# mcan1999/vulkan-raytracing

Measured on AMD Instinct MI355X. Metric: Mrays/sec (primary+secondary) at 1920×1080 depth 4; 1/2/4/8-GPU scaling, higher is better.
Workload: dtype f32

## Files before the change

### vulkan_raytracing_amd/csrc/kernels.hip

```cpp
#include <hip/hip_runtime.h>

#include "rt_kernels.h"

namespace rt {

struct F3 { float x, y, z; };
__device__ __forceinline__ F3 mk3(float x, float y, float z) { F3 r; r.x = x; r.y = y; r.z = z; return r; }
__device__ __forceinline__ F3 add3(F3 a, F3 b) { return mk3(a.x + b.x, a.y + b.y, a.z + b.z); }
__device__ __forceinline__ F3 sub3(F3 a, F3 b) { return mk3(a.x - b.x, a.y - b.y, a.z - b.z); }
__device__ __forceinline__ F3 mul3(F3 a, float s) { return mk3(a.x * s, a.y * s, a.z * s); }
__device__ __forceinline__ F3 neg3(F3 a) { return mk3(-a.x, -a.y, -a.z); }
__device__ __forceinline__ float dot3(F3 a, F3 b) { return __builtin_fmaf(a.z, b.z, __builtin_fmaf(a.y, b.y, a.x * b.x)); }
__device__ __forceinline__ F3 cross3(F3 a, F3 b) {
  return mk3(__builtin_fmaf(a.y, b.z, -(a.z * b.y)), __builtin_fmaf(a.z, b.x, -(a.x * b.z)), __builtin_fmaf(a.x, b.y, -(a.y * b.x)));
}
__device__ __forceinline__ float length3(F3 v) { return __builtin_sqrtf(dot3(v, v)); }
__device__ __forceinline__ F3 normalize3(F3 v) { float inv = 1.0f / length3(v); return mul3(v, inv); }
__device__ __forceinline__ F3 fma3(float s, F3 a, F3 b) { return mk3(__builtin_fmaf(s, a.x, b.x), __builtin_fmaf(s, a.y, b.y), __builtin_fmaf(s, a.z, b.z)); }
__device__ __forceinline__ F3 reflect3(F3 I, F3 N) { float k = 2.0f * dot3(N, I); return fma3(-k, N, I); }

__device__ __forceinline__ F3 xform_point(const float* m, F3 p) {
  return mk3(__builtin_fmaf(m[2], p.z, __builtin_fmaf(m[1], p.y, m[0] * p.x)) + m[3],
             __builtin_fmaf(m[6], p.z, __builtin_fmaf(m[5], p.y, m[4] * p.x)) + m[7],
             __builtin_fmaf(m[10], p.z, __builtin_fmaf(m[9], p.y, m[8] * p.x)) + m[11]);
// ... 1260 lines not shown
      atomicAdd(reinterpret_cast<unsigned long long*>(a.counters + CNT_NODE_VISITS + off), (unsigned long long)cnt_nodes);
      atomicAdd(reinterpret_cast<unsigned long long*>(a.counters + CNT_TRI_TESTS + off), (unsigned long long)cnt_tris);
      const int dg = ANY ? CNT_DIAG_SH : CNT_DIAG;
      atomicAdd(reinterpret_cast<unsigned long long*>(a.counters + dg), (unsigned long long)diag_iters);
      atomicAdd(reinterpret_cast<unsigned long long*>(a.counters + dg + 2), (unsigned long long)diag_busy);
      atomicAdd(reinterpret_cast<unsigned long long*>(a.counters + dg + 4), (unsigned long long)(__builtin_readcyclecounter() - diag_t0));
    }
  }
}

template <int MODE, bool ANY, bool WIDE, bool ENTRY = false, bool FAR = true, bool CONT = false>
__global__ __launch_bounds__(256) __attribute__((amdgpu_waves_per_eu(RT_WAVES_PER_EU, RT_WAVES_PER_EU))) void k_trace(TraceArgs a) { trace_body<MODE, ANY, false, WIDE, ENTRY, FAR, CONT>(a); }
template <int MODE, bool ANY, bool WIDE, bool ENTRY = false, bool FAR = true, bool CONT = false>
__global__ __launch_bounds__(256) void k_trace_count(TraceArgs a) { trace_body<MODE, ANY, true, WIDE, ENTRY, FAR, CONT>(a); }

#include "kernels_beam.inc"

#ifdef RT_ALT_KERNELS
#include "kernels_alt.inc"
#include "kernels_tile.inc"
#endif

struct ShadeArgs {
  SceneDev sc;
  FrameDev f;
  UniformsDev u;
  int bounce;
  BatchTab bt;
};

struct Surface { F3 P, N; };
__device__ __forceinline__ Surface hit_surface(const SceneDev& sc, const InstanceDev* I, uint32_t prim, float hu, float hv) {
  const uint32_t* ix = sc.idx + I->first_index + 3u * prim;
  const uint32_t ia = ix[0], ib = ix[1], ic = ix[2];
  const float* vb = sc.verts + I->first_float;
  const float bx = (1.0f - hu) - hv, by = hu, bz = hv;
  const float* pa = vb + 6u * ia; const float* pb = vb + 6u * ib; const float* pc = vb + 6u * ic;
  const F3 pos = fma3(bz, mk3(pc[0], pc[1], pc[2]), fma3(by, mk3(pb[0], pb[1], pb[2]), mul3(mk3(pa[0], pa[1], pa[2]), bx)));
  const F3 nrm = fma3(bz, mk3(pc[3], pc[4], pc[5]), fma3(by, mk3(pb[3], pb[4], pb[5]), mul3(mk3(pa[3], pa[4], pa[5]), bx)));
  Surface s;
  s.P = xform_point(I->o2w, pos);
  s.N = normalize3(xform_normal(I->w2o, nrm));
  return s;
}

template <bool TILE = false, bool BATCH = false, bool RUNS = false>
__device__ __forceinline__ void shade_body(const ShadeArgs& a, const int bounce) {
  const FrameDev& f = a.f;
  const UniformsDev& U = a.u;
  const int cur = bounce & 1, nxt = cur ^ 1;
  const uint32_t lane = threadIdx.x & 63u, wave = threadIdx.x >> 6;
  const int n_pass = TILE ? 2 : 1;
  for (int pass = 0; pass < n_pass; pass++) {
  uint32_t cnt[N_SHARDS], maxb = 0;
#pragma unroll
  for (int t = 0; t < N_SHARDS; t++) {
    if (TILE && pass) {
      uint32_t blobs = 0;
#pragma unroll
      for (int k = 0; k < BLOB_CLASSES; k++) blobs += ld_cursor(f.counters + cnt_tail(Q_BLOB_LIST + k, t));
      cnt[t] = blobs * (256u * ((U.samples_per_pixel + 3u) / 4u));
    } else cnt[t] = ld_cursor(f.counters + cnt_tail(bounce, t));
    maxb = max(maxb, (cnt[t] + 63u) >> 6);
  }
  const uint32_t n_waves = gridDim.x * 4u;
  for (uint32_t g = blockIdx.x * 4u + wave; g < maxb * N_SHARDS; g += n_waves) {
    const uint32_t shard = g & (N_SHARDS - 1), base = (g >> 3) << 6;
    uint32_t n = 0;
#pragma unroll
    for (int t = 0; t < N_SHARDS; t++) n = (shard == (uint32_t)t) ? cnt[t] : n;
    if (base >= n) continue;
    const uint32_t q = shard * f.shard_cap + ((TILE && pass) ? f.shard_cap - n : 0u) + base + lane;
    bool push_next = false, push_shadow = false, settled = false;
    F3 no = mk3(0, 0, 0), nd = mk3(0, 0, 1);
    float sh_tmax = 0.f; F3 sh_c = mk3(0, 0, 0); float sh_w = 0.f;
    uint32_t sh_ent = ENTRY_FROM_ROOT;
    uint32_t sid = SID_DEAD;
    int inst = HIT_DEAD;
    if (base + lane < n) inst = ld_stream(&f.hit_inst[q]);
    if (inst != HIT_DEAD) {
      const float4 rd = ld_stream(&f.ray_d[cur][q]);
      sid = __float_as_uint(rd.w);
      const F3 d = mk3(rd.x, rd.y, rd.z);
      if (inst < 0) {
        const F3 c = sample_sky(a.sc, mk3(d.x, d.y, -d.z));
        st_stream(&f.sample_color[sid], make_float4(c.x, c.y, c.z, 1.0f));
      } else {
        const float4 h = ld_stream(&f.hit_a[q]);
        const InstanceDev* I = a.sc.inst + inst;
        const uint32_t prim = __float_as_uint(h.w);
        const Surface S = hit_surface(a.sc, I, prim, h.y, h.z);
        const F3 P = S.P;
        F3 N = S.N;
        const int objectIndex = I->custom_index;
        uint32_t type = I->type != TYPE_BY_OBJECT_INDEX ? I->type : (objectIndex == 0 ? U.center_object_type : U.orbiting_object_type);
        const MaterialDev* M = nullptr;
        uint32_t mat = MATERIAL_NONE;
        if (a.sc.n_materials != 0) {
          mat = a.sc.prim_material[I->first_index / 3u + prim];
          M = a.sc.materials + mat;
          if (M->type != TYPE_BY_INSTANCE) type = M->type;
        }
        const bool last = (uint32_t)bounce >= U.max_bounce_count;
        if (type == 0u) {
          if (dot3(d, N) >= 0.0f) {
            st_stream(&f.sample_color[sid], make_float4(0.08f, 0.24f, 0.08f, 1.0f));
          } else {
            no = fma3(0.01f, N, P);
            F3 light = mk3(U.light_position[0], U.light_position[1], U.light_position[2]);
            float Iv = U.light_intensity;
            uint32_t fi = 0;
            if (BATCH) { fi = frame_of(sid, a.sc.batch_samples); light = mk3(a.bt.light[fi][0], a.bt.light[fi][1], a.bt.light[fi][2]); Iv = a.bt.light[fi][3]; }
            const F3 toL = sub3(light, P);
            const float dist = length3(toL);
            const F3 L = mul3(toL, 1.0f / dist);
            const F3 Hh = normalize3(add3(L, neg3(d)));
            const float NdotL = dot3(N, L), NdotH = dot3(N, Hh);
            const float dl = fmaxf(0.0f, NdotL);
            const float sp = M ? pow_int(fmaxf(0.0f, NdotH), (uint32_t)M->ns) : pow100(fmaxf(0.0f, NdotH));
            const uint32_t i = sid / (uint32_t)(f.rows * f.width) - fi * U.samples_per_pixel;
            float w = 1.0f;
            for (uint32_t k = 0; k < i; k++) w = w * 0.9f;
            const F3 kd = M ? mk3(M->kd[0], M->kd[1], M->kd[2]) : mk3(0.2f, 1.0f, 0.2f);
            const F3 ks = M ? mk3(M->ks[0], M->ks[1], M->ks[2]) : mk3(0.8f, 0.8f, 0.8f);
            const F3 diff = mk3((Iv * kd.x) * dl, (Iv * kd.y) * dl, (Iv * kd.z) * dl);
            const F3 spec = mk3((Iv * ks.x) * sp, (Iv * ks.y) * sp, (Iv * ks.z) * sp);
            const F3 amb = ambient_of(a.sc, mat);
            sh_c = fma3(w, add3(diff, spec), amb); sh_w = __uint_as_float(mat);
            nd = L; sh_tmax = dist;
            push_shadow = true;
            if (f.settle_dead_shadow_rays && __float_as_uint(sh_c.x) == __float_as_uint(amb.x) && __float_as_uint(sh_c.y) == __float_as_uint(amb.y) &&
                __float_as_uint(sh_c.z) == __float_as_uint(amb.z)) {
              st_stream(&f.sample_color[sid], make_float4(amb.x, amb.y, amb.z, 1.0f));
              push_shadow = false; settled = true;
            }
            if (f.light_entry != nullptr) {
              const F3 v = sub3(no, light);
              const float ax = __builtin_fabsf(v.x), ay = __builtin_fabsf(v.y), az = __builtin_fabsf(v.z);
              const int axis = (ax >= ay && ax >= az) ? 0 : (ay >= az ? 1 : 2);
              const float vc = axis == 0 ? v.x : (axis == 1 ? v.y : v.z), va = axis == 0 ? v.y : (axis == 1 ? v.z : v.x), vb = axis == 0 ? v.z : (axis == 1 ? v.x : v.y);
              const float c = __builtin_fabsf(vc);
              if (c > 0.0f) {
                const float T8 = (float)(8 * f.light_tiles);
                const float px = (va / c + 1.0f) * 0.5f * T8, py = (1.0f - vb / c) * 0.5f * T8;
                const int tx = min(max((int)(px * 0.125f), 0), f.light_tiles - 1), ty = min(max((int)(py * 0.125f), 0), f.light_tiles - 1);
                const int face = 2 * axis + (vc < 0.0f ? 1 : 0);
                sh_ent = (uint32_t)((face * f.light_tiles + ty) * f.light_tiles + tx) | (NdotL < 0.0f ? ENTRY_REVERSE : 0u);
              }
            }
          }
        } else if (type == 1u) {
          no = fma3(0.01f, N, P);
          nd = reflect3(d, N);
          push_next = true;
        } else if (type == 2u) {
          float ndoti = dot3(d, N);
          const bool outwards = ndoti > 0.0f;
          if (outwards) { N = neg3(N); ndoti = -ndoti; }
          const float ratio = M ? (outwards ? M->ni : 1.0f / M->ni) : (outwards ? 1.52f : (1.0f / 1.52f));
          const float k = 1.0f - (ratio * ratio) * (1.0f - ndoti * ndoti);
          if (k < 0.0f) { nd = reflect3(d, N); no = fma3(0.01f, N, P); }
          else {
            const float c = __builtin_fmaf(ratio, ndoti, __builtin_sqrtf(k));
            nd = normalize3(fma3(-c, N, mul3(d, ratio)));
            no = fma3(-0.01f, N, P);
          }
          push_next = true;
        } else {
          if (bounce == 0 && f.pixel_runs) {
            no = mk3(U.position[0], U.position[1], U.position[2]);
            if (BATCH) { const uint32_t fk = frame_of(sid, a.sc.batch_samples); no = mk3(a.bt.position[fk][0], a.bt.position[fk][1], a.bt.position[fk][2]); }
          } else {
            const float4 ro = ld_stream(&f.ray_o[cur][q]);
            no = mk3(ro.x, ro.y, ro.z);
          }
          nd = d; push_next = true;
        }
        if (push_next && last) {
          push_next = false;
          st_stream(&f.sample_color[sid], make_float4(0.08f, 0.24f, 0.08f, 1.0f));
        }
      }
    }
    {
      const uint64_t m_st = __ballot(settled);
      if (lane == 0 && m_st != 0ull) {
        __hip_atomic_fetch_add(f.counters + cnt_tail(Q_SHADOW0, (int)shard), (uint32_t)__builtin_popcountll(m_st), __ATOMIC_RELAXED, __HIP_MEMORY_SCOPE_AGENT);
        __hip_atomic_fetch_add(f.counters + cnt_work(Q_DEAD, (int)shard), (uint32_t)__builtin_popcountll(m_st), __ATOMIC_RELAXED, __HIP_MEMORY_SCOPE_AGENT);
      }
    }
    const uint32_t slot_n = wave_alloc(push_next, f.counters + cnt_tail(bounce + 1, (int)shard));
    if (push_next) {
      const uint32_t v = shard * f.shard_cap + slot_n;
      st_stream(&f.ray_o[nxt][v], make_float4(no.x, no.y, no.z, 10000.0f));
      st_stream(&f.ray_d[nxt][v], make_float4(nd.x, nd.y, nd.z, __uint_as_float(sid)));
    }
    if (RUNS) {
      if (base + lane < n) {
        if (push_shadow) {
          st_stream(&f.sh_o[q], make_float4(no.x, no.y, no.z, sh_tmax));
          st_stream(&f.sh_c[q], make_float4(sh_c.x, sh_c.y, sh_c.z, sh_w));
          if (f.sh_e != nullptr) f.sh_e[q] = sh_ent;
        }
        st_stream(&f.sh_d[q], push_shadow ? make_float4(nd.x, nd.y, nd.z, __uint_as_float(sid)) : make_float4(0.f, 0.f, 0.f, __uint_as_float(SID_DEAD)));
      }
      const uint64_t m_sh = __ballot(push_shadow);
      if (lane == 0 && m_sh != 0ull) __hip_atomic_fetch_add(f.counters + cnt_tail(Q_SHADOW0, (int)shard), (uint32_t)__builtin_popcountll(m_sh), __ATOMIC_RELAXED, __HIP_MEMORY_SCOPE_AGENT);
    } else {
      const uint32_t slot_s = wave_alloc(push_shadow, f.counters + cnt_tail(Q_SHADOW, (int)shard));
      if (push_shadow) {
        const uint32_t v = f.sh_base + shard * f.shard_cap + slot_s;
        st_stream(&f.sh_o[v], make_float4(no.x, no.y, no.z, sh_tmax));
        st_stream(&f.sh_d[v], make_float4(nd.x, nd.y, nd.z, __uint_as_float(sid)));
        st_stream(&f.sh_c[v], make_float4(sh_c.x, sh_c.y, sh_c.z, sh_w));
        if (f.sh_e != nullptr) f.sh_e[v] = sh_ent;
      }
    }
  }
  }
}

template <bool TILE, bool BATCH, bool RUNS = false>
__global__ __launch_bounds__(256) void k_shade(ShadeArgs a) { shade_body<TILE, BATCH, RUNS>(a, a.bounce); }

struct TailArgs {
  TraceArgs tr;
  ShadeArgs sh;
  uint32_t first_bounce;
  uint32_t* barrier;
  uint32_t* fault;
};

__device__ __forceinline__ void grid_barrier(uint32_t* bar, uint32_t* fault, uint32_t& phase) {
  __syncthreads();
  phase++;
  if (threadIdx.x == 0) {
    __threadfence();
    const uint32_t target = phase * gridDim.x;
// ... 200 lines not shown
    a.rays_per_lane = (uint32_t)cfg.rays_per_lane; a.min_blocks = (uint32_t)cfg.min_blocks;
    const dim3 g(cfg.trace_blocks), b(256);
#ifdef RT_ALT_KERNELS
    if (f.tile_blob != nullptr) {
      if (counting) hipLaunchKernelGGL((k_trace_count<MODE_CLOSEST, false, false, true, false, true>), g, b, 0, s, a);
      else hipLaunchKernelGGL((k_trace<MODE_CLOSEST, false, false, true, false, true>), g, b, 0, s, a);
      return;
    }
#endif
    if (counting) hipLaunchKernelGGL((k_trace_count<MODE_CLOSEST, false, false, true>), g, b, 0, s, a);
    else if (cfg.far) hipLaunchKernelGGL((k_trace<MODE_CLOSEST, false, false, true, true>), g, b, 0, s, a);
    else hipLaunchKernelGGL((k_trace<MODE_CLOSEST, false, false, true, false>), g, b, 0, s, a);
    return;
  }
  launch_trace<MODE_CLOSEST, false>(a, counting, cfg, s);
}

void launch_entry(const SceneDev& sc, const EntryViews& a, hipStream_t s) {
  uint32_t n = 0;
  for (int v = 0; v < a.n; v++) n = max(n, (uint32_t)(a.v[v].tiles_x * a.v[v].tile_rows));
  if (n == 0) return;
  hipLaunchKernelGGL(k_entry, dim3((n + 7u) / 8u, (unsigned)a.n), dim3(64), 0, s, sc, a);
}

void launch_trace_shadow(const SceneDev& sc, const FrameDev& f, bool counting, const LaunchCfg& cfg, hipStream_t s) {
  TraceArgs a = make_args(sc, f.counters, Q_SHADOW, f.shard_cap, f.ovf_stack);
  a.ray_o = f.sh_o + f.sh_base; a.ray_d = f.sh_d + f.sh_base; a.sh_c = f.sh_c + f.sh_base;
  a.sample_color = f.sample_color;
#ifdef RT_ALT_KERNELS
  if (cfg.packet != 0 && cfg.variant == 0) {
// ... 303 lines not shown
```

### vulkan_raytracing_amd/csrc/kernels_beam.inc

```
struct BeamSpace { F3 s0, b0, s1, b1; uint3 rot; };

__device__ __forceinline__ bool slab_beam(uint32_t wx, uint32_t wy, uint32_t wz, const BeamSpace& B, float tmin, float tlim, float& tn) {
  wx = __builtin_amdgcn_alignbit(wx, wx, B.rot.x); wy = __builtin_amdgcn_alignbit(wy, wy, B.rot.y); wz = __builtin_amdgcn_alignbit(wz, wz, B.rot.z);
  const float nx = (float)(wx & 0xFFFFu), fx = (float)(wx >> 16), ny = (float)(wy & 0xFFFFu), fy = (float)(wy >> 16), nz = (float)(wz & 0xFFFFu), fz = (float)(wz >> 16);
  const float x0 = fminf(__builtin_fmaf(nx, B.s0.x, B.b0.x), __builtin_fmaf(nx, B.s1.x, B.b1.x)), x1 = fmaxf(__builtin_fmaf(fx, B.s0.x, B.b0.x), __builtin_fmaf(fx, B.s1.x, B.b1.x));
  const float y0 = fminf(__builtin_fmaf(ny, B.s0.y, B.b0.y), __builtin_fmaf(ny, B.s1.y, B.b1.y)), y1 = fmaxf(__builtin_fmaf(fy, B.s0.y, B.b0.y), __builtin_fmaf(fy, B.s1.y, B.b1.y));
  const float z0 = fminf(__builtin_fmaf(nz, B.s0.z, B.b0.z), __builtin_fmaf(nz, B.s1.z, B.b1.z)), z1 = fmaxf(__builtin_fmaf(fz, B.s0.z, B.b0.z), __builtin_fmaf(fz, B.s1.z, B.b1.z));
  tn = fmaxf(fmaxf(x0, y0), fmaxf(z0, tmin));
  const float tf = fminf(fminf(x1, y1), fminf(z1, tlim));
  return tn <= tf * 1.00002f;
}
__device__ __forceinline__ void beam_axis(float lo, float hi, float da, float t_far, float q_lo_minus_o, float q_scale, float& s0, float& b0, float& s1, float& b1, uint32_t& rot) {
  if (lo < 0.0f && hi > 0.0f) {
    const float K = 1.0e30f, inv = 1.0f / q_scale, r = t_far * da;
    const float U = (r - q_lo_minus_o) * inv + 1.0f, L = (-r - q_lo_minus_o) * inv - 1.0f;
    s0 = K; s1 = K; b0 = -K * U; b1 = -K * L; rot = 0u;
  }
  else { s0 = q_scale * lo; b0 = q_lo_minus_o * lo; s1 = q_scale * hi; b1 = q_lo_minus_o * hi; rot = lo < 0.0f ? 16u : 0u; }
}

#define RT_BEAM_EACH(M) M(0) M(1) M(2) M(3)
#ifndef RT_BEAM_KEEP_NUM
#define RT_BEAM_KEEP_NUM RT_KEEP_NUM
#endif
#ifndef RT_BEAM_UNROLL
#define RT_BEAM_UNROLL RT_INTERIOR_UNROLL
#endif

template <bool COUNT>
__device__ __forceinline__ void beam_body(const TraceArgs& a, const uint32_t run) {
  __shared__ int s_stack[4][STACK2_LDS + 1][64];
  __shared__ float s_best[4][16][64];
  __shared__ float4 s_inst[LDS_INSTANCES ? LDS_INSTANCES : 1][5];
  const int n_lds_inst = a.sc.n_inst < LDS_INSTANCES ? a.sc.n_inst : LDS_INSTANCES;
  if ((int)threadIdx.x < n_lds_inst) {
    const InstanceDev* I = a.sc.inst + threadIdx.x;
    const float4* mp = reinterpret_cast<const float4*>(I->w2o);
    s_inst[threadIdx.x][0] = mp[0]; s_inst[threadIdx.x][1] = mp[1]; s_inst[threadIdx.x][2] = mp[2];
    s_inst[threadIdx.x][3] = make_float4(I->q_lo[0], I->q_lo[1], I->q_lo[2], __int_as_float(I->blas_root));
    s_inst[threadIdx.x][4] = make_float4(I->q_scale[0], I->q_scale[1], I->q_scale[2], __uint_as_float(I->mask));
  }
  __syncthreads();
  const uint32_t lane = threadIdx.x & 63u, wave = threadIdx.x >> 6;
  int* const stk = &s_stack[wave][0][lane];
  float* const bst = &s_best[wave][0][lane];
// ... 197 lines not shown
          push(REF_MARK);
          cur_inst = ii; cur = root;
        }
      }
    }

    if (COUNT) {
      uint32_t mx = my_visits;
      for (int off = 32; off > 0; off >>= 1) mx = max(mx, (uint32_t)__shfl_xor((int)mx, off));
      if (lane == 0) {
        atomicMax(a.counters + CNT_TILE_DIAG, mx);
        atomicAdd(reinterpret_cast<unsigned long long*>(a.counters + CNT_TILE_DIAG + 2), (unsigned long long)mx);
        atomicAdd(reinterpret_cast<unsigned long long*>(a.counters + CNT_TILE_DIAG + 4), 1ull);
      }
    }
#define RT_BEAM_OUT(j) if (j < S) { \
      const uint32_t v = v0 + 64u * j; \
      if (alive & (1u << j)) { \
        st_stream(&a.hit_a[v], make_float4(bt##j, bst[(4 * j + 0) * 64], bst[(4 * j + 1) * 64], bst[(4 * j + 2) * 64])); \
        st_stream(&a.hit_inst[v], __float_as_int(bst[(4 * j + 3) * 64])); \
      } else st_stream(&a.hit_inst[v], HIT_DEAD); }
    RT_BEAM_EACH(RT_BEAM_OUT)
#undef RT_BEAM_OUT
  }
  if (COUNT) {
    for (int off = 32; off > 0; off >>= 1) {
      cnt_nodes += __shfl_down((unsigned long long)cnt_nodes, off);
      cnt_tris += __shfl_down((unsigned long long)cnt_tris, off);
    }
    if (lane == 0) {
      atomicAdd(reinterpret_cast<unsigned long long*>(a.counters + CNT_NODE_VISITS), (unsigned long long)cnt_nodes);
      atomicAdd(reinterpret_cast<unsigned long long*>(a.counters + CNT_TRI_TESTS), (unsigned long long)cnt_tris);
      atomicAdd(reinterpret_cast<unsigned long long*>(a.counters + CNT_DIAG), (unsigned long long)diag_iters);
      atomicAdd(reinterpret_cast<unsigned long long*>(a.counters + CNT_DIAG + 2), (unsigned long long)diag_busy);
      atomicAdd(reinterpret_cast<unsigned long long*>(a.counters + CNT_DIAG + 4), (unsigned long long)(__builtin_readcyclecounter() - diag_t0));
    }
  }
}

#ifndef RT_BEAM_WAVES
#define RT_BEAM_WAVES 4
#endif
__global__ __launch_bounds__(256) __attribute__((amdgpu_waves_per_eu(RT_BEAM_WAVES, RT_BEAM_WAVES))) void k_beam(TraceArgs a, uint32_t run) { beam_body<false>(a, run); }
__global__ __launch_bounds__(256) void k_beam_count(TraceArgs a, uint32_t run) { beam_body<true>(a, run); }

#ifdef RT_ALT_KERNELS
struct BeamShadowArgs {
  TraceArgs t;
  float light[3];
  uint32_t run;
};
struct BeamSpaceW { F3 s0, s1, n0, n1, f0, f1; uint3 rot; };

__device__ __forceinline__ bool slab_beam_w(uint32_t wx, uint32_t wy, uint32_t wz, const BeamSpaceW& B, float tmin, float tlim, float& tn, float& tfo) {
  wx = __builtin_amdgcn_alignbit(wx, wx, B.rot.x); wy = __builtin_amdgcn_alignbit(wy, wy, B.rot.y); wz = __builtin_amdgcn_alignbit(wz, wz, B.rot.z);
  const float nx = (float)(wx & 0xFFFFu), fx = (float)(wx >> 16), ny = (float)(wy & 0xFFFFu), fy = (float)(wy >> 16), nz = (float)(wz & 0xFFFFu), fz = (float)(wz >> 16);
  const float x0 = fminf(__builtin_fmaf(nx, B.s0.x, B.n0.x), __builtin_fmaf(nx, B.s1.x, B.n1.x)), x1 = fmaxf(__builtin_fmaf(fx, B.s0.x, B.f0.x), __builtin_fmaf(fx, B.s1.x, B.f1.x));
  const float y0 = fminf(__builtin_fmaf(ny, B.s0.y, B.n0.y), __builtin_fmaf(ny, B.s1.y, B.n1.y)), y1 = fmaxf(__builtin_fmaf(fy, B.s0.y, B.f0.y), __builtin_fmaf(fy, B.s1.y, B.f1.y));
  const float z0 = fminf(__builtin_fmaf(nz, B.s0.z, B.n0.z), __builtin_fmaf(nz, B.s1.z, B.n1.z)), z1 = fmaxf(__builtin_fmaf(fz, B.s0.z, B.f0.z), __builtin_fmaf(fz, B.s1.z, B.f1.z));
// ... 279 lines not shown
```

### vulkan_raytracing_amd/csrc/rt_api.cpp

```cpp
#include "../../include/rt_api.h"

#include <hip/hip_runtime.h>

#include <algorithm>
#include <cmath>
#include <cstdio>
#include <cstring>
#include <map>
#include <mutex>
#include <queue>
#include <string>
#include <vector>

#include "blas_refit.h"
#include "bvh_build.h"
#include "bvh_gpu.h"
#include "rt_device.h"
#include "rt_kernels.h"
#include "tlas_gpu.h"

using namespace rt;

static_assert(sizeof(rt_instance) == 64, "rt_instance must mirror VkAccelerationStructureInstanceKHR (64 B)");
static_assert(sizeof(rt_uniforms) == 104, "rt_uniforms must mirror UniformStructure (104 B)");
// ... 159 lines not shown
  int jitter_table = 1;
  const float2* jitter_waited = nullptr; hipStream_t jitter_waited_stream = nullptr;
  int primary_cover = 1;
  int tail_min_blocks = 1;
  bool tail_full_grid = false;
  int entry_max_instances = 32;
  int entry_points = 1;
  int shadow_entry = 2;
  int light_tiles = LIGHT_TILES_DEFAULT;
  EntryRec* d_entry = nullptr;
  size_t entry_alloc_tiles = 0;
  int camera_records = 1;
  int dead_shadow_rays = 1;
  int shadow_beams = 0;
  bool sh_double = false;
  int pixel_beams = 1;
  int tile_blobs = 0;
  uint32_t* d_tile_blob = nullptr;
  char* d_blob_arena = nullptr;
  uint32_t blob_slots = 0;
  uint4* d_blob_list = nullptr;
  size_t tile_dir_alloc = 0;
  EntryRec* d_light_entry = nullptr;
  size_t light_alloc_tiles = 0;
  uint32_t* d_cover_mask = nullptr;
  uint32_t cover_alloc_words = 0;
  int cover_parity = 0;
  unsigned long long* h_stats = nullptr;
  unsigned long long* d_stats = nullptr;
  bool last_empty = false;
// ... 841 lines not shown
  {
    Span frame_span(c, CAT_FRAME, s);
    {
      Span sp(c, CAT_RAYGEN, s);
      if (f.cover) launch_cover(sc, cv, c->scene->max_cover_count, const_cast<uint32_t*>(f.cover), s);
      if (f.entry || ev.n > 1) launch_entry(sc, ev, s);
      if (f.tile_blob) launch_blob(sc, ev.v[0], f, c->counting, s);
      launch_raygen(sc, f, u, bt, s);
    }
    uint32_t tail_start = 0xFFFFFFFFu;
    const bool tail_ok = c->cfg.variant != 1 && c->tail_blocks > 0 && !no_tail && !c->tail_disabled;
    if (tail_ok && c->tail_mode == 2) tail_start = 1;
    else if (tail_ok && c->tail_mode == 1)
      for (uint32_t b = 1; b <= u.max_bounce_count && b < (uint32_t)CNT_MAX_BOUNCES; b++)
        if (((volatile uint32_t*)c->h_hint)[b] <= TAIL_MAX_RAYS) { tail_start = b; break; }
    for (uint32_t b = 0; b <= u.max_bounce_count; b++) {
      if (b == tail_start) {
        int tb = std::min(c->tail_blocks, tail_grid(c->n_cu, c->tail_resident_per_cu, live_slots_on(c->device)));
        if (tb <= 0) { { Span sp(c, CAT_TRACE, s); launch_trace_closest(sc, f, (int)b, c->counting, cfg, s); } { Span sp(c, CAT_SHADE, s); launch_shade(sc, f, u, bt, (int)b, cfg, s); } continue; }
        const uint32_t expect = ((volatile uint32_t*)c->h_hint)[b];
        if (c->tail_mode == 1 && expect != 0xFFFFFFFFu && !c->tail_full_grid && c->scene->members.size() >= 3) {
          long want = ((long)expect + 255) / 256;
          const long lo = c->tail_min_blocks;
          if (lo >= N_SHARDS) want = (want + (N_SHARDS - 1)) / N_SHARDS * N_SHARDS;
          tb = (int)std::min<long>(tb, std::max<long>(lo, want));
        }
        Span sp(c, CAT_TAIL, s); launch_tail(sc, f, u, bt, (int)b, c->counting, cfg, tb, s);
        break;
      }
      { LaunchCfg cc = cfg; if (b == 0 && cap_closest > 0) cc.trace_blocks = std::min(cfg.trace_blocks, c->n_cu * cap_closest);
        Span sp(c, CAT_TRACE, s);
        if (b == 0 && f.tile_blob) launch_tile(sc, f, u, c->counting, s);
        launch_trace_closest(sc, f, (int)b, c->counting, cc, s); }
      { Span sp(c, CAT_SHADE, s); launch_shade(sc, f, u, bt, (int)b, cfg, s); }
      if (b >= 7 && (b & 3) == 3 && b < u.max_bounce_count) {
        uint32_t tails[N_SHARDS * CNT_STRIDE];
        HIP_TRY(c, hipMemcpyAsync(tails, f.counters + cnt_tail((int)b + 1, 0), sizeof(tails), hipMemcpyDeviceToHost, s));
        HIP_TRY(c, hipStreamSynchronize(s));
        uint32_t live = 0;
        for (int t = 0; t < N_SHARDS; t++) live += tails[t * CNT_STRIDE];
        if (live == 0) break;
      }
    }
    { LaunchCfg cs = cfg; if (cap_shadow > 0) cs.trace_blocks = std::min(cfg.trace_blocks, c->n_cu * cap_shadow);
      Span sp(c, CAT_SHADOW, s); launch_beam_shadow(sc, f, u, c->counting, cs, s); launch_trace_shadow(sc, f, c->counting, cs, s); }
    { Span sp(c, CAT_RESOLVE, s); launch_resolve(f, u, s); }
  }
  HIP_TRY(c, hipGetLastError());
  if (!c->ev_frame[frame_parity]) HIP_TRY(c, hipEventCreateWithFlags(&c->ev_frame[frame_parity], hipEventDisableTiming));
// ... 587 lines not shown
    if (c->async_pending) return fail(c, RT_ERR_NOT_READY, "output_rgba8 cannot change while a frame is pending");
    c->out_rgba8 = value != 0; c->out_bgra = false; return RT_OK;
  }
  if (k == "output_bgra8") {
    if (value != 0 && value != 1) return fail(c, RT_ERR_INVALID_ARGUMENT, "output_bgra8 must be 0 or 1");
    if (c->async_pending) return fail(c, RT_ERR_NOT_READY, "output_bgra8 cannot change while a frame is pending");
    c->out_rgba8 = value != 0; c->out_bgra = value != 0; return RT_OK;
  }
  if (k == "primary_cover") { c->primary_cover = value != 0; return RT_OK; }
  if (k == "jitter_table") { c->jitter_table = value != 0; return RT_OK; }
  if (k == "tile_blobs") {
    if (value != 0 && !alt_kernels_built()) return fail(c, RT_ERR_INVALID_ARGUMENT, "tile_blobs is not in the product library (measured slower): build librt_mi355x_alt.so with `make alt` and load it (RT_LIB_VARIANT=alt)");
    c->tile_blobs = value != 0; return RT_OK;
  }
  if (k == "pixel_beams") { c->pixel_beams = value != 0; return RT_OK; }
  if (k == "camera_records") { c->camera_records = value != 0; return RT_OK; }
  if (k == "dead_shadow_rays") { c->dead_shadow_rays = value != 0; return RT_OK; }
  if (k == "shadow_beams") {
    if (value != 0 && !alt_kernels_built()) return fail(c, RT_ERR_INVALID_ARGUMENT, "shadow_beams is not in the product library (measured slower): build librt_mi355x_alt.so with `make alt` and load it (RT_LIB_VARIANT=alt)");
    c->shadow_beams = value != 0; return RT_OK;
  }

  if (k == "entry_points") { c->entry_points = value != 0; return RT_OK; }
  if (k == "packet_trace") {
    if (value < 0 || value > 2) return fail(c, RT_ERR_INVALID_ARGUMENT, "packet_trace must be 0, 1 or 2");
    if (value != 0 && !alt_kernels_built()) return fail(c, RT_ERR_INVALID_ARGUMENT, "packet_trace is not in the product library (measured slower): build librt_mi355x_alt.so with `make alt` and load it (RT_LIB_VARIANT=alt)");
    c->cfg.packet = value; return RT_OK;
  }
  if (k == "packet_blocks_per_cu") { if (value < 1 || value > 16) return fail(c, RT_ERR_INVALID_ARGUMENT, "packet_blocks_per_cu must be 1..16"); c->cfg.packet_blocks = c->n_cu * value; return RT_OK; }
  if (k == "shadow_entry") { if (value < 0 || value > 2) return fail(c, RT_ERR_INVALID_ARGUMENT, "shadow_entry must be 0, 1 or 2"); if (value != c->shadow_entry) { c->light_built = false; c->light_seen_valid = false; } c->shadow_entry = value; return RT_OK; }
// ... 635 lines not shown
```

### vulkan_raytracing_amd/csrc/rt_kernels.h

```cpp
#pragma once
#include <hip/hip_runtime.h>
#include <stdint.h>

#include "rt_device.h"

namespace rt {

struct SceneDev {
  const BvhNodeQ* blas_nodes;
  int tlas_root;
  int tlas_nodes;
  int tlas_stride;
  uint32_t batch_samples;
  const float4* tris;
  float tlas_q_lo[3], tlas_q_scale[3];
  const WideNodeQ* wide_nodes;
  const Bvh4Node* nodes4;
  int tlas_root4;
  const InstanceDev* inst;
  const float* verts;
  const uint32_t* idx;
  const uchar4* sky;
  int n_inst;
  int sky_w, sky_h;
// ... 85 lines not shown
  int trace_blocks;
  int shade_blocks;
  int rays_per_lane;
  int min_blocks;
  int variant;
  int far;
  int packet;
  int packet_blocks;
};

size_t raygen_block_count(int width, int rows, uint32_t spp, int batch_k);
void launch_raygen(const SceneDev& sc, const FrameDev& f, const UniformsDev& u, const BatchTab& bt, hipStream_t s);
size_t jitter_table_elems(int width, int rows, uint32_t spp);
void launch_jitter_table(const FrameDev& f, uint32_t spp, float2* table, hipStream_t s);
void launch_trace_closest(const SceneDev& sc, const FrameDev& f, int bounce, bool counting, const LaunchCfg& cfg, hipStream_t s);
void launch_entry(const SceneDev& sc, const EntryViews& a, hipStream_t s);
void launch_blob(const SceneDev& sc, const EntryArgs& e, const FrameDev& f, bool counting, hipStream_t s);
void launch_tile(const SceneDev& sc, const FrameDev& f, const UniformsDev& u, bool counting, hipStream_t s);
void launch_tail(const SceneDev& sc, const FrameDev& f, const UniformsDev& u, const BatchTab& bt, int first_bounce, bool counting, const LaunchCfg& cfg, int tail_blocks, hipStream_t s);
void launch_shade(const SceneDev& sc, const FrameDev& f, const UniformsDev& u, const BatchTab& bt, int bounce, const LaunchCfg& cfg, hipStream_t s);
void launch_beam_shadow(const SceneDev& sc, const FrameDev& f, const UniformsDev& u, bool counting, const LaunchCfg& cfg, hipStream_t s);
void launch_trace_shadow(const SceneDev& sc, const FrameDev& f, bool counting, const LaunchCfg& cfg, hipStream_t s);
void launch_resolve(const FrameDev& f, const UniformsDev& u, hipStream_t s);
void launch_cover(const SceneDev& sc, const CoverViews& a, uint32_t max_boxes_per_instance, uint32_t* mask_block, hipStream_t s);
void launch_query(const SceneDev& sc, const float4* rays, HitRec* out, uint32_t n, int32_t* ovf_stack, uint32_t* counters, bool any_hit,
                  bool counting, const LaunchCfg& cfg, hipStream_t s);
void launch_hit_attr(const SceneDev& sc, const HitRec* hits, float4* attr, uint32_t n, hipStream_t s);
void launch_query_flags(const SceneDev& sc, const float4* rays, const uint32_t* words, uint32_t query_word, HitRec* out, uint32_t n,
                        int32_t* ovf_stack, uint32_t* counters, const LaunchCfg& cfg, hipStream_t s);
void launch_hit_kind(const SceneDev& sc, const float4* rays, const HitRec* hits, float4* attr, uint32_t n, hipStream_t s);
// ... 21 lines not shown
```

Measured before the change: 32340.

## Fuse primary-ray shading into the beam trace kernel for bounce zero

Pulls the per-ray shading logic out into a reusable shade_slot helper and calls it directly from the beam traversal kernel for primary rays. Hit instance and barycentrics are passed in registers, so hit records are no longer written to and read back from global memory, and the separate shade launch for bounce 0 is skipped. The path is on by default when beams, camera records and single-frame conditions hold. In exchange the beam kernel gets more register pressure and code size, which may lower occupancy, and the shading loop runs serialized per slot inside the beam.

```diff
diff --git a/vulkan_raytracing_amd/csrc/kernels.hip b/vulkan_raytracing_amd/csrc/kernels.hip
--- a/vulkan_raytracing_amd/csrc/kernels.hip
+++ b/vulkan_raytracing_amd/csrc/kernels.hip
@@ -1298,8 +1298,6 @@
 template <int MODE, bool ANY, bool WIDE, bool ENTRY = false, bool FAR = true, bool CONT = false>
 __global__ __launch_bounds__(256) void k_trace_count(TraceArgs a) { trace_body<MODE, ANY, true, WIDE, ENTRY, FAR, CONT>(a); }
 
-#include "kernels_beam.inc"
-
 #ifdef RT_ALT_KERNELS
 #include "kernels_alt.inc"
 #include "kernels_tile.inc"
@@ -1328,11 +1326,169 @@
   return s;
 }
 
+template <bool PIN> __device__ __forceinline__ float4 ambient_default() {
+  float r = 0.08f;
+  if constexpr (PIN) asm volatile("" : "+v"(r));
+  return make_float4(r, 0.24f, r, 1.0f);
+}
+template <bool TILE, bool BATCH, bool RUNS, bool REG, typename A>
+__device__ __forceinline__ void shade_slot(const A& a, const int bounce, const uint32_t shard, const uint32_t q, const bool in_range, const int inst_r, const float4 h_r) {
+  const auto& f = a.f;
+  const auto& U = a.u;
+  const int cur = bounce & 1, nxt = cur ^ 1;
+  const uint32_t lane = threadIdx.x & 63u;
+  bool push_next = false, push_shadow = false, settled = false;
+  F3 no = mk3(0, 0, 0), nd = mk3(0, 0, 1);
+  float sh_tmax = 0.f; F3 sh_c = mk3(0, 0, 0); float sh_w = 0.f;
+  uint32_t sh_ent = ENTRY_FROM_ROOT;
+  uint32_t sid = SID_DEAD;
+  int inst = HIT_DEAD;
+  if (in_range) { if constexpr (REG) inst = inst_r; else inst = ld_stream(&f.hit_inst[q]); }
+  if (inst != HIT_DEAD) {
+    const float4 rd = ld_stream(&f.ray_d[cur][q]);
+    sid = __float_as_uint(rd.w);
+    const F3 d = mk3(rd.x, rd.y, rd.z);
+    if (inst < 0) {
+      const F3 c = sample_sky(a.sc, mk3(d.x, d.y, -d.z));
+      st_stream(&f.sample_color[sid], make_float4(c.x, c.y, c.z, 1.0f));
+    } else {
+      float4 h = h_r;
+      if constexpr (!REG) h = ld_stream(&f.hit_a[q]);
+      const InstanceDev* I = a.sc.inst + inst;
+      const uint32_t prim = __float_as_uint(h.w);
+      const Surface S = hit_surface(a.sc, I, prim, h.y, h.z);
+      const F3 P = S.P;
+      F3 N = S.N;
+      const int objectIndex = I->custom_index;
+      uint32_t type = I->type != TYPE_BY_OBJECT_INDEX ? I->type : (objectIndex == 0 ? U.center_object_type : U.orbiting_object_type);
+      const MaterialDev* M = nullptr;
+      uint32_t mat = MATERIAL_NONE;
+      if (a.sc.n_materials != 0) {
+        mat = a.sc.prim_material[I->first_index / 3u + prim];
+        M = a.sc.materials + mat;
+        if (M->type != TYPE_BY_INSTANCE) type = M->type;
+      }
+      const bool last = (uint32_t)bounce >= U.max_bounce_count;
+      if (type == 0u) {
+        if (dot3(d, N) >= 0.0f) {
+          st_stream(&f.sample_color[sid], ambient_default<REG>());
+        } else {
+          no = fma3(0.01f, N, P);
+          F3 light = mk3(U.light_position[0], U.light_position[1], U.light_position[2]);
+          float Iv = U.light_intensity;
+          uint32_t fi = 0;
+          if constexpr (BATCH) { fi = frame_of(sid, a.sc.batch_samples); light = mk3(a.bt.light[fi][0], a.bt.light[fi][1], a.bt.light[fi][2]); Iv = a.bt.light[fi][3]; }
+          const F3 toL = sub3(light, P);
+          const float dist = length3(toL);
+          const F3 L = mul3(toL, 1.0f / dist);
+          const F3 Hh = normalize3(add3(L, neg3(d)));
+          const float NdotL = dot3(N, L), NdotH = dot3(N, Hh);
+          const float dl = fmaxf(0.0f, NdotL);
+          const float sp = M ? pow_int(fmaxf(0.0f, NdotH), (uint32_t)M->ns) : pow100(fmaxf(0.0f, NdotH));
+          const uint32_t i = sid / (uint32_t)(f.rows * f.width) - fi * U.samples_per_pixel;
+          float w = 1.0f;
+          for (uint32_t k = 0; k < i; k++) w = w * 0.9f;
+          const F3 kd = M ? mk3(M->kd[0], M->kd[1], M->kd[2]) : mk3(0.2f, 1.0f, 0.2f);
+          const F3 ks = M ? mk3(M->ks[0], M->ks[1], M->ks[2]) : mk3(0.8f, 0.8f, 0.8f);
+          const F3 diff = mk3((Iv * kd.x) * dl, (Iv * kd.y) * dl, (Iv * kd.z) * dl);
+          const F3 spec = mk3((Iv * ks.x) * sp, (Iv * ks.y) * sp, (Iv * ks.z) * sp);
+          const F3 amb = ambient_of(a.sc, mat);
+          sh_c = fma3(w, add3(diff, spec), amb); sh_w = __uint_as_float(mat);
+          nd = L; sh_tmax = dist;
+          push_shadow = true;
+          if (f.settle_dead_shadow_rays && __float_as_uint(sh_c.x) == __float_as_uint(amb.x) && __float_as_uint(sh_c.y) == __float_as_uint(amb.y) &&
+              __float_as_uint(sh_c.z) == __float_as_uint(amb.z)) {
+            st_stream(&f.sample_color[sid], make_float4(amb.x, amb.y, amb.z, 1.0f));
+            push_shadow = false; settled = true;
+          }
+          if (f.light_entry != nullptr) {
+            const F3 v = sub3(no, light);
+            const float ax = __builtin_fabsf(v.x), ay = __builtin_fabsf(v.y), az = __builtin_fabsf(v.z);
+            const int axis = (ax >= ay && ax >= az) ? 0 : (ay >= az ? 1 : 2);
+            const float vc = axis == 0 ? v.x : (axis == 1 ? v.y : v.z), va = axis == 0 ? v.y : (axis == 1 ? v.z : v.x), vb = axis == 0 ? v.z : (axis == 1 ? v.x : v.y);
+            const float c = __builtin_fabsf(vc);
+            if (c > 0.0f) {
+              const float T8 = (float)(8 * f.light_tiles);
+              const float px = (va / c + 1.0f) * 0.5f * T8, py = (1.0f - vb / c) * 0.5f * T8;
+              const int tx = min(max((int)(px * 0.125f), 0), f.light_tiles - 1), ty = min(max((int)(py * 0.125f), 0), f.light_tiles - 1);
+              const int face = 2 * axis + (vc < 0.0f ? 1 : 0);
+              sh_ent = (uint32_t)((face * f.light_tiles + ty) * f.light_tiles + tx) | (NdotL < 0.0f ? ENTRY_REVERSE : 0u);
+            }
+          }
+        }
+      } else if (type == 1u) {
+        no = fma3(0.01f, N, P);
+        nd = reflect3(d, N);
+        push_next = true;
+      } else if (type == 2u) {
+        float ndoti = dot3(d, N);
+        const bool outwards = ndoti > 0.0f;
+        if (outwards) { N = neg3(N); ndoti = -ndoti; }
+        const float ratio = M ? (outwards ? M->ni : 1.0f / M->ni) : (outwards ? 1.52f : (1.0f / 1.52f));
+        const float k = 1.0f - (ratio * ratio) * (1.0f - ndoti * ndoti);
+        if (k < 0.0f) { nd = reflect3(d, N); no = fma3(0.01f, N, P); }
+        else {
+          const float c = __builtin_fmaf(ratio, ndoti, __builtin_sqrtf(k));
+          nd = normalize3(fma3(-c, N, mul3(d, ratio)));
+          no = fma3(-0.01f, N, P);
+        }
+        push_next = true;
+      } else {
+        if (bounce == 0 && f.pixel_runs) {
+          no = mk3(U.position[0], U.position[1], U.position[2]);
+          if constexpr (BATCH) { const uint32_t fk = frame_of(sid, a.sc.batch_samples); no = mk3(a.bt.position[fk][0], a.bt.position[fk][1], a.bt.position[fk][2]); }
+        } else {
+          const float4 ro = ld_stream(&f.ray_o[cur][q]);
+          no = mk3(ro.x, ro.y, ro.z);
+        }
+        nd = d; push_next = true;
+      }
+      if (push_next && last) {
+        push_next = false;
+        st_stream(&f.sample_color[sid], ambient_default<REG>());
+      }
+    }
+  }
+  {
+    const uint64_t m_st = __ballot(settled);
+    if (lane == 0 && m_st != 0ull) {
+      __hip_atomic_fetch_add(f.counters + cnt_tail(Q_SHADOW0, (int)shard), (uint32_t)__builtin_popcountll(m_st), __ATOMIC_RELAXED, __HIP_MEMORY_SCOPE_AGENT);
+      __hip_atomic_fetch_add(f.counters + cnt_work(Q_DEAD, (int)shard), (uint32_t)__builtin_popcountll(m_st), __ATOMIC_RELAXED, __HIP_MEMORY_SCOPE_AGENT);
+    }
+  }
+  const uint32_t slot_n = wave_alloc(push_next, f.counters + cnt_tail(bounce + 1, (int)shard));
+  if (push_next) {
+    const uint32_t v = shard * f.shard_cap + slot_n;
+    st_stream(&f.ray_o[nxt][v], make_float4(no.x, no.y, no.z, 10000.0f));
+    st_stream(&f.ray_d[nxt][v], make_float4(nd.x, nd.y, nd.z, __uint_as_float(sid)));
+  }
+  if constexpr (RUNS) {
+    if (in_range) {
+      if (push_shadow) {
+        st_stream(&f.sh_o[q], make_float4(no.x, no.y, no.z, sh_tmax));
+        st_stream(&f.sh_c[q], make_float4(sh_c.x, sh_c.y, sh_c.z, sh_w));
+        if (f.sh_e != nullptr) f.sh_e[q] = sh_ent;
+      }
+      st_stream(&f.sh_d[q], push_shadow ? make_float4(nd.x, nd.y, nd.z, __uint_as_float(sid)) : make_float4(0.f, 0.f, 0.f, __uint_as_float(SID_DEAD)));
+    }
+    const uint64_t m_sh = __ballot(push_shadow);
+    if (lane == 0 && m_sh != 0ull) __hip_atomic_fetch_add(f.counters + cnt_tail(Q_SHADOW0, (int)shard), (uint32_t)__builtin_popcountll(m_sh), __ATOMIC_RELAXED, __HIP_MEMORY_SCOPE_AGENT);
+  } else {
+    const uint32_t slot_s = wave_alloc(push_shadow, f.counters + cnt_tail(Q_SHADOW, (int)shard));
+    if (push_shadow) {
+      const uint32_t v = f.sh_base + shard * f.shard_cap + slot_s;
+      st_stream(&f.sh_o[v], make_float4(no.x, no.y, no.z, sh_tmax));
+      st_stream(&f.sh_d[v], make_float4(nd.x, nd.y, nd.z, __uint_as_float(sid)));
+      st_stream(&f.sh_c[v], make_float4(sh_c.x, sh_c.y, sh_c.z, sh_w));
+      if (f.sh_e != nullptr) f.sh_e[v] = sh_ent;
+    }
+  }
+}
+
 template <bool TILE = false, bool BATCH = false, bool RUNS = false>
 __device__ __forceinline__ void shade_body(const ShadeArgs& a, const int bounce) {
   const FrameDev& f = a.f;
   const UniformsDev& U = a.u;
-  const int cur = bounce & 1, nxt = cur ^ 1;
   const uint32_t lane = threadIdx.x & 63u, wave = threadIdx.x >> 6;
   const int n_pass = TILE ? 2 : 1;
   for (int pass = 0; pass < n_pass; pass++) {
@@ -1355,157 +1511,15 @@
     for (int t = 0; t < N_SHARDS; t++) n = (shard == (uint32_t)t) ? cnt[t] : n;
     if (base >= n) continue;
     const uint32_t q = shard * f.shard_cap + ((TILE && pass) ? f.shard_cap - n : 0u) + base + lane;
-    bool push_next = false, push_shadow = false, settled = false;
-    F3 no = mk3(0, 0, 0), nd = mk3(0, 0, 1);
-    float sh_tmax = 0.f; F3 sh_c = mk3(0, 0, 0); float sh_w = 0.f;
-    uint32_t sh_ent = ENTRY_FROM_ROOT;
-    uint32_t sid = SID_DEAD;
-    int inst = HIT_DEAD;
-    if (base + lane < n) inst = ld_stream(&f.hit_inst[q]);
-    if (inst != HIT_DEAD) {
-      const float4 rd = ld_stream(&f.ray_d[cur][q]);
-      sid = __float_as_uint(rd.w);
-      const F3 d = mk3(rd.x, rd.y, rd.z);
-      if (inst < 0) {
-        const F3 c = sample_sky(a.sc, mk3(d.x, d.y, -d.z));
-        st_stream(&f.sample_color[sid], make_float4(c.x, c.y, c.z, 1.0f));
-      } else {
-        const float4 h = ld_stream(&f.hit_a[q]);
-        const InstanceDev* I = a.sc.inst + inst;
-        const uint32_t prim = __float_as_uint(h.w);
-        const Surface S = hit_surface(a.sc, I, prim, h.y, h.z);
-        const F3 P = S.P;
-        F3 N = S.N;
-        const int objectIndex = I->custom_index;
-        uint32_t type = I->type != TYPE_BY_OBJECT_INDEX ? I->type : (objectIndex == 0 ? U.center_object_type : U.orbiting_object_type);
-        const MaterialDev* M = nullptr;
-        uint32_t mat = MATERIAL_NONE;
-        if (a.sc.n_materials != 0) {
-          mat = a.sc.prim_material[I->first_index / 3u + prim];
-          M = a.sc.materials + mat;
-          if (M->type != TYPE_BY_INSTANCE) type = M->type;
-        }
-        const bool last = (uint32_t)bounce >= U.max_bounce_count;
-        if (type == 0u) {
-          if (dot3(d, N) >= 0.0f) {
-            st_stream(&f.sample_color[sid], make_float4(0.08f, 0.24f, 0.08f, 1.0f));
-          } else {
-            no = fma3(0.01f, N, P);
-            F3 light = mk3(U.light_position[0], U.light_position[1], U.light_position[2]);
-            float Iv = U.light_intensity;
-            uint32_t fi = 0;
-            if (BATCH) { fi = frame_of(sid, a.sc.batch_samples); light = mk3(a.bt.light[fi][0], a.bt.light[fi][1], a.bt.light[fi][2]); Iv = a.bt.light[fi][3]; }
-            const F3 toL = sub3(light, P);
-            const float dist = length3(toL);
-            const F3 L = mul3(toL, 1.0f / dist);
-            const F3 Hh = normalize3(add3(L, neg3(d)));
-            const float NdotL = dot3(N, L), NdotH = dot3(N, Hh);
-            const float dl = fmaxf(0.0f, NdotL);
-            const float sp = M ? pow_int(fmaxf(0.0f, NdotH), (uint32_t)M->ns) : pow100(fmaxf(0.0f, NdotH));
-            const uint32_t i = sid / (uint32_t)(f.rows * f.width) - fi * U.samples_per_pixel;
-            float w = 1.0f;
-            for (uint32_t k = 0; k < i; k++) w = w * 0.9f;
-            const F3 kd = M ? mk3(M->kd[0], M->kd[1], M->kd[2]) : mk3(0.2f, 1.0f, 0.2f);
-            const F3 ks = M ? mk3(M->ks[0], M->ks[1], M->ks[2]) : mk3(0.8f, 0.8f, 0.8f);
-            const F3 diff = mk3((Iv * kd.x) * dl, (Iv * kd.y) * dl, (Iv * kd.z) * dl);
-            const F3 spec = mk3((Iv * ks.x) * sp, (Iv * ks.y) * sp, (Iv * ks.z) * sp);
-            const F3 amb = ambient_of(a.sc, mat);
-            sh_c = fma3(w, add3(diff, spec), amb); sh_w = __uint_as_float(mat);
-            nd = L; sh_tmax = dist;
-            push_shadow = true;
-            if (f.settle_dead_shadow_rays && __float_as_uint(sh_c.x) == __float_as_uint(amb.x) && __float_as_uint(sh_c.y) == __float_as_uint(amb.y) &&
-                __float_as_uint(sh_c.z) == __float_as_uint(amb.z)) {
-              st_stream(&f.sample_color[sid], make_float4(amb.x, amb.y, amb.z, 1.0f));
-              push_shadow = false; settled = true;
-            }
-            if (f.light_entry != nullptr) {
-              const F3 v = sub3(no, light);
-              const float ax = __builtin_fabsf(v.x), ay = __builtin_fabsf(v.y), az = __builtin_fabsf(v.z);
-              const int axis = (ax >= ay && ax >= az) ? 0 : (ay >= az ? 1 : 2);
-              const float vc = axis == 0 ? v.x : (axis == 1 ? v.y : v.z), va = axis == 0 ? v.y : (axis == 1 ? v.z : v.x), vb = axis == 0 ? v.z : (axis == 1 ? v.x : v.y);
-              const float c = __builtin_fabsf(vc);
-              if (c > 0.0f) {
-                const float T8 = (float)(8 * f.light_tiles);
-                const float px = (va / c + 1.0f) * 0.5f * T8, py = (1.0f - vb / c) * 0.5f * T8;
-                const int tx = min(max((int)(px * 0.125f), 0), f.light_tiles - 1), ty = min(max((int)(py * 0.125f), 0), f.light_tiles - 1);
-                const int face = 2 * axis + (vc < 0.0f ? 1 : 0);
-                sh_ent = (uint32_t)((face * f.light_tiles + ty) * f.light_tiles + tx) | (NdotL < 0.0f ? ENTRY_REVERSE : 0u);
-              }
-            }
-          }
-        } else if (type == 1u) {
-          no = fma3(0.01f, N, P);
-          nd = reflect3(d, N);
-          push_next = true;
-        } else if (type == 2u) {
-          float ndoti = dot3(d, N);
-          const bool outwards = ndoti > 0.0f;
-          if (outwards) { N = neg3(N); ndoti = -ndoti; }
-          const float ratio = M ? (outwards ? M->ni : 1.0f / M->ni) : (outwards ? 1.52f : (1.0f / 1.52f));
-          const float k = 1.0f - (ratio * ratio) * (1.0f - ndoti * ndoti);
-          if (k < 0.0f) { nd = reflect3(d, N); no = fma3(0.01f, N, P); }
-          else {
-            const float c = __builtin_fmaf(ratio, ndoti, __builtin_sqrtf(k));
-            nd = normalize3(fma3(-c, N, mul3(d, ratio)));
-            no = fma3(-0.01f, N, P);
-          }
-          push_next = true;
-        } else {
-          if (bounce == 0 && f.pixel_runs) {
-            no = mk3(U.position[0], U.position[1], U.position[2]);
-            if (BATCH) { const uint32_t fk = frame_of(sid, a.sc.batch_samples); no = mk3(a.bt.position[fk][0], a.bt.position[fk][1], a.bt.position[fk][2]); }
-          } else {
-            const float4 ro = ld_stream(&f.ray_o[cur][q]);
-            no = mk3(ro.x, ro.y, ro.z);
-          }
-          nd = d; push_next = true;
-        }
-        if (push_next && last) {
-          push_next = false;
-          st_stream(&f.sample_color[sid], make_float4(0.08f, 0.24f, 0.08f, 1.0f));
-        }
-      }
-    }
-    {
-      const uint64_t m_st = __ballot(settled);
-      if (lane == 0 && m_st != 0ull) {
-        __hip_atomic_fetch_add(f.counters + cnt_tail(Q_SHADOW0, (int)shard), (uint32_t)__builtin_popcountll(m_st), __ATOMIC_RELAXED, __HIP_MEMORY_SCOPE_AGENT);
-        __hip_atomic_fetch_add(f.counters + cnt_work(Q_DEAD, (int)shard), (uint32_t)__builtin_popcountll(m_st), __ATOMIC_RELAXED, __HIP_MEMORY_SCOPE_AGENT);
-      }
-    }
-    const uint32_t slot_n = wave_alloc(push_next, f.counters + cnt_tail(bounce + 1, (int)shard));
-    if (push_next) {
-      const uint32_t v = shard * f.shard_cap + slot_n;
-      st_stream(&f.ray_o[nxt][v], make_float4(no.x, no.y, no.z, 10000.0f));
-      st_stream(&f.ray_d[nxt][v], make_float4(nd.x, nd.y, nd.z, __uint_as_float(sid)));
-    }
-    if (RUNS) {
-      if (base + lane < n) {
-        if (push_shadow) {
-          st_stream(&f.sh_o[q], make_float4(no.x, no.y, no.z, sh_tmax));
-          st_stream(&f.sh_c[q], make_float4(sh_c.x, sh_c.y, sh_c.z, sh_w));
-          if (f.sh_e != nullptr) f.sh_e[q] = sh_ent;
-        }
-        st_stream(&f.sh_d[q], push_shadow ? make_float4(nd.x, nd.y, nd.z, __uint_as_float(sid)) : make_float4(0.f, 0.f, 0.f, __uint_as_float(SID_DEAD)));
-      }
-      const uint64_t m_sh = __ballot(push_shadow);
-      if (lane == 0 && m_sh != 0ull) __hip_atomic_fetch_add(f.counters + cnt_tail(Q_SHADOW0, (int)shard), (uint32_t)__builtin_popcountll(m_sh), __ATOMIC_RELAXED, __HIP_MEMORY_SCOPE_AGENT);
-    } else {
-      const uint32_t slot_s = wave_alloc(push_shadow, f.counters + cnt_tail(Q_SHADOW, (int)shard));
-      if (push_shadow) {
-        const uint32_t v = f.sh_base + shard * f.shard_cap + slot_s;
-        st_stream(&f.sh_o[v], make_float4(no.x, no.y, no.z, sh_tmax));
-        st_stream(&f.sh_d[v], make_float4(nd.x, nd.y, nd.z, __uint_as_float(sid)));
-        st_stream(&f.sh_c[v], make_float4(sh_c.x, sh_c.y, sh_c.z, sh_w));
-        if (f.sh_e != nullptr) f.sh_e[v] = sh_ent;
-      }
-    }
+    shade_slot<TILE, BATCH, RUNS, false>(a, bounce, shard, q, base + lane < n, HIT_DEAD, make_float4(0.f, 0.f, 0.f, 0.f));
   }
   }
 }
 
 template <bool TILE, bool BATCH, bool RUNS = false>
 __global__ __launch_bounds__(256) void k_shade(ShadeArgs a) { shade_body<TILE, BATCH, RUNS>(a, a.bounce); }
+
+#include "kernels_beam.inc"
 
 struct TailArgs {
   TraceArgs tr;
@@ -1736,6 +1750,26 @@
     return;
   }
   launch_trace<MODE_CLOSEST, false>(a, counting, cfg, s);
+}
+
+void launch_beam_shade(const SceneDev& sc, const FrameDev& f, const UniformsDev& u, const LaunchCfg& cfg, hipStream_t s) {
+  BeamShadeArgs a{};
+  a.sc = sc;
+  a.ray_o = f.ray_o[0]; a.ray_d = f.ray_d[0];
+  a.tails = f.counters + cnt_tail(0, 0); a.work = f.counters + cnt_work(0, 0);
+  a.shard_cap = f.shard_cap; a.ovf_stack = f.ovf_stack; a.counters = f.counters;
+  a.tmin = 0.001f;
+  a.entry = f.entry;
+  a.next_o = f.ray_o[1]; a.next_d = f.ray_d[1];
+  a.sh_o = f.sh_o; a.sh_d = f.sh_d; a.sh_c = f.sh_c; a.sh_e = f.sh_e;
+  a.sample_color = f.sample_color;
+  a.light_entry = f.light_entry;
+  a.width = f.width; a.rows = f.rows; a.light_tiles = f.light_tiles; a.settle_dead_shadow_rays = f.settle_dead_shadow_rays;
+  for (int k = 0; k < 3; k++) { a.u.position[k] = u.position[k]; a.u.light_position[k] = u.light_position[k]; }
+  a.u.light_intensity = u.light_intensity;
+  a.u.max_bounce_count = u.max_bounce_count; a.u.samples_per_pixel = u.samples_per_pixel;
+  a.u.center_object_type = u.center_object_type; a.u.orbiting_object_type = u.orbiting_object_type;
+  hipLaunchKernelGGL(k_beam_shade, dim3(cfg.trace_blocks), dim3(256), 0, s, a, (uint32_t)f.pixel_runs);
 }
 
 void launch_entry(const SceneDev& sc, const EntryViews& a, hipStream_t s) {
diff --git a/vulkan_raytracing_amd/csrc/kernels_beam.inc b/vulkan_raytracing_amd/csrc/kernels_beam.inc
--- a/vulkan_raytracing_amd/csrc/kernels_beam.inc
+++ b/vulkan_raytracing_amd/csrc/kernels_beam.inc
@@ -27,8 +27,47 @@
 #define RT_BEAM_UNROLL RT_INTERIOR_UNROLL
 #endif
 
-template <bool COUNT>
-__device__ __forceinline__ void beam_body(const TraceArgs& a, const uint32_t run) {
+struct BeamShadeUniforms {
+  float position[3], light_position[3], light_intensity;
+  uint32_t max_bounce_count, samples_per_pixel, center_object_type, orbiting_object_type;
+};
+struct BeamShadeArgs {
+  SceneDev sc;
+  const float4* ray_o;
+  const float4* ray_d;
+  const uint32_t* tails;
+  uint32_t* work;
+  uint32_t shard_cap;
+  int32_t* ovf_stack;
+  uint32_t* counters;
+  float tmin;
+  const EntryRec* entry;
+  float4* next_o;
+  float4* next_d;
+  float4* sh_o;
+  float4* sh_d;
+  float4* sh_c;
+  uint32_t* sh_e;
+  float4* sample_color;
+  const EntryRec* light_entry;
+  int width, rows, light_tiles, settle_dead_shadow_rays;
+  BeamShadeUniforms u;
+};
+struct BeamShadeFrame {
+  float4* ray_o[2]; float4* ray_d[2];
+  float4* sh_o; float4* sh_d; float4* sh_c; uint32_t* sh_e;
+  float4* sample_color;
+  uint32_t* counters;
+  const EntryRec* light_entry;
+  uint32_t shard_cap;
+  int width, rows, light_tiles, settle_dead_shadow_rays;
+  static constexpr int pixel_runs = 64;
+  static constexpr uint32_t sh_base = 0u;
+};
+struct BeamShadeView { const SceneDev& sc; const BeamShadeFrame& f; const BeamShadeUniforms& u; };
+
+template <bool COUNT, bool SHADE = false, typename Args = TraceArgs>
+__device__ __forceinline__ void beam_body(const Args& a, const uint32_t run) {
   __shared__ int s_stack[4][STACK2_LDS + 1][64];
   __shared__ float s_best[4][16][64];
   __shared__ float4 s_inst[LDS_INSTANCES ? LDS_INSTANCES : 1][5];
@@ -256,6 +295,21 @@
         atomicAdd(reinterpret_cast<unsigned long long*>(a.counters + CNT_TILE_DIAG + 4), 1ull);
       }
     }
+    if constexpr (SHADE) {
+      const uint32_t run_shard = (uint32_t)__builtin_amdgcn_readfirstlane((int)shard);
+      const BeamShadeArgs* ka = (const BeamShadeArgs*)__builtin_amdgcn_kernarg_segment_ptr();
+      asm volatile("" : "+s"(ka));
+      const BeamShadeFrame sf{{const_cast<float4*>(ka->ray_o), ka->next_o}, {const_cast<float4*>(ka->ray_d), ka->next_d}, ka->sh_o, ka->sh_d, ka->sh_c, ka->sh_e, ka->sample_color,
+                              ka->counters, ka->light_entry, ka->shard_cap, ka->width, ka->rows, ka->light_tiles, ka->settle_dead_shadow_rays};
+      const BeamShadeView sv{ka->sc, sf, ka->u};
+#pragma nounroll
+      for (uint32_t j = 0; j < S; j++) {
+        const float tj = j == 0u ? bt0 : (j == 1u ? bt1 : (j == 2u ? bt2 : bt3));
+        const float* const b = bst + 256u * j;
+        const int ij = (alive >> j) & 1u ? __float_as_int(b[192]) : HIT_DEAD;
+        shade_slot<false, false, false, true>(sv, 0, run_shard, v0 + 64u * j, true, ij, make_float4(tj, b[0], b[64], b[128]));
+      }
+    } else {
 #define RT_BEAM_OUT(j) if (j < S) { \
       const uint32_t v = v0 + 64u * j; \
       if (alive & (1u << j)) { \
@@ -264,6 +318,7 @@
       } else st_stream(&a.hit_inst[v], HIT_DEAD); }
     RT_BEAM_EACH(RT_BEAM_OUT)
 #undef RT_BEAM_OUT
+    }
   }
   if (COUNT) {
     for (int off = 32; off > 0; off >>= 1) {
@@ -285,6 +340,7 @@
 #endif
 __global__ __launch_bounds__(256) __attribute__((amdgpu_waves_per_eu(RT_BEAM_WAVES, RT_BEAM_WAVES))) void k_beam(TraceArgs a, uint32_t run) { beam_body<false>(a, run); }
 __global__ __launch_bounds__(256) void k_beam_count(TraceArgs a, uint32_t run) { beam_body<true>(a, run); }
+__global__ __launch_bounds__(256) __attribute__((amdgpu_waves_per_eu(RT_BEAM_WAVES, RT_BEAM_WAVES))) void k_beam_shade(BeamShadeArgs a, uint32_t run) { beam_body<false, true>(a, run); }
 
 #ifdef RT_ALT_KERNELS
 struct BeamShadowArgs {
diff --git a/vulkan_raytracing_amd/csrc/rt_api.cpp b/vulkan_raytracing_amd/csrc/rt_api.cpp
--- a/vulkan_raytracing_amd/csrc/rt_api.cpp
+++ b/vulkan_raytracing_amd/csrc/rt_api.cpp
@@ -197,6 +197,7 @@
   int dead_shadow_rays = 1;
   int shadow_beams = 0;
   bool sh_double = false;
+  int fused_shade = 1;
   int pixel_beams = 1;
   int tile_blobs = 0;
   uint32_t* d_tile_blob = nullptr;
@@ -1068,6 +1069,7 @@
     else if (tail_ok && c->tail_mode == 1)
       for (uint32_t b = 1; b <= u.max_bounce_count && b < (uint32_t)CNT_MAX_BOUNCES; b++)
         if (((volatile uint32_t*)c->h_hint)[b] <= TAIL_MAX_RAYS) { tail_start = b; break; }
+    const bool fused0 = c->fused_shade && beam_on && c->camera_records && K == 1 && !c->counting && !f.tile_blob && !f.shadow_runs && tail_start != 0u;
     for (uint32_t b = 0; b <= u.max_bounce_count; b++) {
       if (b == tail_start) {
         int tb = std::min(c->tail_blocks, tail_grid(c->n_cu, c->tail_resident_per_cu, live_slots_on(c->device)));
@@ -1085,8 +1087,9 @@
       { LaunchCfg cc = cfg; if (b == 0 && cap_closest > 0) cc.trace_blocks = std::min(cfg.trace_blocks, c->n_cu * cap_closest);
         Span sp(c, CAT_TRACE, s);
         if (b == 0 && f.tile_blob) launch_tile(sc, f, u, c->counting, s);
-        launch_trace_closest(sc, f, (int)b, c->counting, cc, s); }
-      { Span sp(c, CAT_SHADE, s); launch_shade(sc, f, u, bt, (int)b, cfg, s); }
+        if (b == 0 && fused0) launch_beam_shade(sc, f, u, cc, s);
+        else launch_trace_closest(sc, f, (int)b, c->counting, cc, s); }
+      if (!(b == 0 && fused0)) { Span sp(c, CAT_SHADE, s); launch_shade(sc, f, u, bt, (int)b, cfg, s); }
       if (b >= 7 && (b & 3) == 3 && b < u.max_bounce_count) {
         uint32_t tails[N_SHARDS * CNT_STRIDE];
         HIP_TRY(c, hipMemcpyAsync(tails, f.counters + cnt_tail((int)b + 1, 0), sizeof(tails), hipMemcpyDeviceToHost, s));
@@ -1704,6 +1707,7 @@
     c->tile_blobs = value != 0; return RT_OK;
   }
   if (k == "pixel_beams") { c->pixel_beams = value != 0; return RT_OK; }
+  if (k == "fused_shade") { c->fused_shade = value != 0; return RT_OK; }
   if (k == "camera_records") { c->camera_records = value != 0; return RT_OK; }
   if (k == "dead_shadow_rays") { c->dead_shadow_rays = value != 0; return RT_OK; }
   if (k == "shadow_beams") {
diff --git a/vulkan_raytracing_amd/csrc/rt_kernels.h b/vulkan_raytracing_amd/csrc/rt_kernels.h
--- a/vulkan_raytracing_amd/csrc/rt_kernels.h
+++ b/vulkan_raytracing_amd/csrc/rt_kernels.h
@@ -123,6 +123,7 @@
 size_t jitter_table_elems(int width, int rows, uint32_t spp);
 void launch_jitter_table(const FrameDev& f, uint32_t spp, float2* table, hipStream_t s);
 void launch_trace_closest(const SceneDev& sc, const FrameDev& f, int bounce, bool counting, const LaunchCfg& cfg, hipStream_t s);
+void launch_beam_shade(const SceneDev& sc, const FrameDev& f, const UniformsDev& u, const LaunchCfg& cfg, hipStream_t s);
 void launch_entry(const SceneDev& sc, const EntryViews& a, hipStream_t s);
 void launch_blob(const SceneDev& sc, const EntryArgs& e, const FrameDev& f, bool counting, hipStream_t s);
 void launch_tile(const SceneDev& sc, const FrameDev& f, const UniformsDev& u, bool counting, hipStream_t s);
```

Result: faster. 34920 (median of 6 runs) (+8.0%).
